# ChaissonLab/LRA

Measured on AMD Instinct MI355X. Metric: aligned Gbp/s, 30 kb ONT vs GRCh38 (MapRead_lowacc end to end incl. SAM text), per job, higher is better.
Workload: dtype int32

## Files before the change

### lra_amd/csrc/sdp.h

```cpp
#pragma once
#include "common.h"
#include <vector>

namespace lra_sdp {

constexpr int LV = 18;
constexpr uint32_t NONE = 0xFFFFFFFFu;
constexpr int MAXALN = 16;
constexpr int PEN_TAB_WG = 4096, PEN_TAB_WAVE = 2048;
constexpr int TRACE_CAP = 2560;

struct PwlTab { long long stops[25]; float slope[25], inter[25]; int c1, c2; };

struct Ent { long long val; int b; float v; };
struct Node {
  uint32_t dBase;
  uint32_t nD, nE;
  int32_t last;
  uint32_t sTop, nBlk;
  uint32_t stkOff, blkOff;
  uint32_t stkCap, blkCap;
  long long eLast;
};

struct ReadArena { uint64_t base; uint32_t entOff, apOff, stkOff, visOff, blkPair, poolPair, poolPairs, edOff, visPl; };

struct PtArgs {
  uint64_t nc;
  const uint64_t* cluster_off; const uint64_t* c_start; const uint32_t* c_count; const int32_t* c_strand;
  const uint32_t* q; const uint32_t* t; const int32_t* len;
  const uint32_t* clusRead; const uint64_t* clusFragOff; const uint64_t* clusPtOff; const uint64_t* fragOff; const uint64_t* ptOff;
  const float* rate_in; float rate; int single;
  uint32_t* fq; uint32_t* ft; int32_t* flen; uint32_t* fcl; uint32_t* fai; float* fval; uint32_t* fprevNode; uint32_t* fprevInd; uint8_t* fflags;
  uint8_t* used; uint8_t* fstrand;
  const uint32_t* qe; const uint32_t* te; uint32_t* fqe; uint32_t* fte;
  uint64_t* key1; uint32_t* pay1; uint32_t* iq; uint32_t* it; uint8_t* ifl; uint32_t* ifr; uint32_t* ptRead;
};

struct BuildArgs {
  int r0, n;
  const uint32_t* order;
  const uint64_t* ptOff;
  const uint32_t* hq; const uint32_t* ht; const uint8_t* hfl; const uint32_t* h2; const uint64_t* key3; const uint32_t* pay3;
  uint32_t* scratch;
  uint32_t* cntEntries; uint32_t* cntNodes; uint32_t* cntD; uint32_t* cntV; uint32_t* cntRC;
  uint32_t* lines;
  const ReadArena* ra;
  uint32_t* status;
  unsigned long long* stat;
};

struct ProcArgs {
  int r0, n;
  const uint32_t* order;
  const uint64_t* ptOff; const uint64_t* fragOff;
  const uint8_t* hfl; const uint32_t* hfr;
  const int32_t* flen; float* fval; uint32_t* fprevNode; uint32_t* fprevInd; uint8_t* fflags;
  const float* rate_in; float rate;
  const ReadArena* ra; uint32_t* poolUsed;
  uint32_t* status;
  PwlTab pwl;
  const short* penTab; int penN;
  int dbg;
  int wgNoRing;
  char* wgScratch; const uint64_t* wgOff;
  unsigned long long* stat;
};

struct TraceArgs {
  int r0, n, numAln, single; float alnthres;
  int boxes, globalK; const uint32_t* fqe; const uint32_t* fte; const int32_t* numAnchors; int32_t* chainNum;
  const uint64_t* fragOff; const uint64_t* read_off;
  const uint32_t* fq; const uint32_t* ft; const int32_t* flen; const uint32_t* fcl; const uint32_t* fai;
  const float* fval; const uint32_t* fpred; const uint8_t* fflags; const uint32_t* opay;
  uint8_t* used;
  const ReadArena* ra;
  uint32_t* nChains; uint64_t* chainStart; uint32_t* chainLen; uint32_t* chainBox; float* chainValue;
  uint32_t* ccl; uint32_t* can; uint8_t* clink; uint32_t* cq; uint32_t* ct; int32_t* clen; uint8_t* cstrand; const uint8_t* fstrand;
  const uint32_t* status;
};

namespace {
__device__ __forceinline__ void wave_sync() {
  __builtin_amdgcn_fence(__ATOMIC_RELEASE, "workgroup");
// ... 124 lines not shown
```

### lra_amd/csrc/sdp.hip

```cpp
#include "sdp.h"
#include "scan.h"
#include <algorithm>
#include <cmath>
#include <cstring>
#include <cstdlib>
#include <vector>

using namespace lra_sdp;

namespace {

inline size_t sz(size_t n, size_t elem) { return (n * elem + 255) / 256 * 256; }
inline char* take(char*& w, size_t n, size_t e) { char* p = w; w += sz(n, e); return p; }
#define SDP_TRY(call) do { const int rc__ = (call); if (rc__) return rc__; } while (0)

static long sdp_big_points(const lra_ctx* ctx, int mode) {
  if (const char* e = getenv("LRA_SDP_BIG_POINTS")) return atol(e);
  if (ctx->sdp_inner) return 1500;
  if (mode == 0) return 2500;
  return ctx->pipelined ? 14000 : 6000;
}

int pwl_table(Call& c) {
  lra_ctx* ctx = c.ctx; hipStream_t st = c.st; const lra_sdp_opts* opts = c.opts; PwlTab& pw = c.pw;
// ... 41 lines not shown
  c.fragOff = (uint64_t*)take(wa, n1, 8); c.ptOff = (uint64_t*)take(wa, n1, 8);
  c.status = (uint32_t*)take(wa, n1, 4); c.nChains = (uint32_t*)take(wa, n1, 4);
  c.chainStart = (uint64_t*)take(wa, nslot, 8); c.chainLen = (uint32_t*)take(wa, nslot, 4); c.chainValue = (float*)take(wa, nslot, 4);
  c.chainBox = (uint32_t*)take(wa, 4 * nslot, 4);
  c.chainNum = (int32_t*)take(wa, nslot, 4);
  LRA_HIP_CHECK(ctx, hipMemsetAsync(c.chainLen, 0, nslot * 4, st));
  if (NC > 0) {
    lra_time_begin(ctx, ctx->sdp_inner ? "sdp_inner_points" : "sdp_points");
    launch_cluster_counts(st, NC, c.boxes ? nullptr : c.d_c_count, c.clusFragCnt, c.clusPtCnt, opts->mode == LRA_SDP_SINGLE_CLUSTER);
    lra_time_end(ctx);
  }
  SDP_TRY(lra_exclusive_scan<uint32_t>(ctx, (long)NC, c.clusFragCnt, c.clusFragOff));
  SDP_TRY(lra_exclusive_scan<uint32_t>(ctx, (long)NC, c.clusPtCnt, c.clusPtOff));
  launch_read_offsets(st, n_reads, c.d_cluster_off, c.clusFragOff, c.clusPtOff, c.fragOff, c.ptOff, c.clusRead, c.status, c.nChains);
  c.h_frag.resize(n1); c.h_pt.resize(n1);
  LRA_HIP_CHECK(ctx, hipMemcpyAsync(c.h_frag.data(), c.fragOff, n1 * 8, hipMemcpyDeviceToHost, st));
  LRA_HIP_CHECK(ctx, hipMemcpyAsync(c.h_pt.data(), c.ptOff, n1 * 8, hipMemcpyDeviceToHost, st));
  LRA_HIP_CHECK(ctx, hipStreamSynchronize(st));
  const uint64_t NF = c.NF = c.h_frag[n_reads], NP = c.NP = c.h_pt[n_reads];
  out->n_frags = NF; out->n_points = NP;
  size_t needF = sz(NF + 1, 4) * 16 + sz(2 * NF + 2, 4) + sz(NF + 1, 1) * 5 + sz(NF + 1, 8) * 2 + 4096;
  char* wf = (char*)lra_ensure(ctx, 8, needF);
  if (!wf) return LRA_ERR_NOMEM;
  c.fq = (uint32_t*)take(wf, NF + 1, 4); c.ft = (uint32_t*)take(wf, NF + 1, 4); c.flen = (int32_t*)take(wf, NF + 1, 4);
  c.fcl = (uint32_t*)take(wf, NF + 1, 4); c.fai = (uint32_t*)take(wf, NF + 1, 4); c.fval = (float*)take(wf, NF + 1, 4);
  c.fprevNode = (uint32_t*)take(wf, NF + 1, 4); c.fprevInd = (uint32_t*)take(wf, NF + 1, 4);
  c.ccl = (uint32_t*)take(wf, NF + 1, 4); c.can = (uint32_t*)take(wf, NF + 1, 4);
  c.fflags = (uint8_t*)take(wf, NF + 1, 1); c.used = (uint8_t*)take(wf, NF + 1, 1); c.clink = (uint8_t*)take(wf, NF + 1, 1);
  c.fstrand = (uint8_t*)take(wf, NF + 1, 1); c.cstrand = (uint8_t*)take(wf, NF + 1, 1);
  c.cq = (uint32_t*)take(wf, NF + 1, 4); c.ct = (uint32_t*)take(wf, NF + 1, 4); c.clen = (int32_t*)take(wf, NF + 1, 4);
  c.okey = (uint64_t*)take(wf, NF + 1, 8);
  c.fqe = (uint32_t*)take(wf, NF + 1, 4); c.fte = (uint32_t*)take(wf, NF + 1, 4);
  size_t needP = sz(NP + 1, 8) * 3 + sz(NP + 1, 4) * 11 + sz(NP + 1, 1) * 2 + sz(NF + 1, 4) * 2 + 4096;
  char* wp = (char*)lra_ensure(ctx, 9, needP);
  if (!wp) return LRA_ERR_NOMEM;
  c.key1 = (uint64_t*)take(wp, NP + 1, 8); c.key2 = (uint64_t*)take(wp, NP + 1, 8); c.key3 = (uint64_t*)take(wp, NP + 1, 8);
  c.pay1 = (uint32_t*)take(wp, NP + 1, 4); c.pay2 = (uint32_t*)take(wp, NP + 1, 4); c.pay3 = (uint32_t*)take(wp, NP + 1, 4);
  c.iq = (uint32_t*)take(wp, NP + 1, 4); c.it = (uint32_t*)take(wp, NP + 1, 4); c.ifr = (uint32_t*)take(wp, NP + 1, 4);
  c.ptRead = (uint32_t*)take(wp, NP + 1, 4);
  c.hq = (uint32_t*)take(wp, NP + 1, 4); c.ht = (uint32_t*)take(wp, NP + 1, 4); c.hfr = (uint32_t*)take(wp, NP + 1, 4);
  c.spare = (uint32_t*)take(wp, NP + 1, 4);
  c.ifl = (uint8_t*)take(wp, NP + 1, 1); c.hfl = (uint8_t*)take(wp, NP + 1, 1);
  c.opay = (uint32_t*)take(wp, NF + 1, 4); c.fragRead = (uint32_t*)take(wp, NF + 1, 4);
  out->d_n_chains = c.nChains; out->d_chain_start = c.chainStart; out->d_chain_len = c.chainLen; out->d_chain_box = c.chainBox; out->d_chain_value = c.chainValue;
  out->d_chain_cluster = c.ccl; out->d_chain_anchor = c.can; out->d_chain_link = c.clink; out->d_chain_q = c.cq; out->d_chain_t = c.ct; out->d_chain_alen = c.clen;
  out->d_chain_strand = c.cstrand; out->d_frag_off = c.fragOff; out->d_frag_val = c.fval; out->d_status = c.status;
  out->d_chain_num_anchors = c.boxes ? c.chainNum : nullptr;
  return LRA_OK;
}

void make_points(const Call& c) {
  lra_ctx* ctx = c.ctx; const lra_sdp_opts* opts = c.opts;
  PtArgs pa;
  pa.nc = c.NC; pa.cluster_off = c.d_cluster_off; pa.c_start = c.d_c_start; pa.c_count = c.d_c_count; pa.c_strand = c.d_c_strand; pa.q = c.d_q; pa.t = c.d_t; pa.len = c.d_len;
  pa.clusRead = c.clusRead; pa.clusFragOff = c.clusFragOff; pa.clusPtOff = c.clusPtOff; pa.fragOff = c.fragOff; pa.ptOff = c.ptOff; pa.rate_in = c.d_rate; pa.rate = opts->rate; pa.single = opts->mode == LRA_SDP_SINGLE_CLUSTER;
  pa.fq = c.fq; pa.ft = c.ft; pa.flen = c.flen; pa.fcl = c.fcl; pa.fai = c.fai; pa.fval = c.fval; pa.fprevNode = c.fprevNode; pa.fprevInd = c.fprevInd; pa.fflags = c.fflags; pa.used = c.used; pa.fstrand = c.fstrand;
  pa.qe = c.d_qe; pa.te = c.d_te; pa.fqe = c.fqe; pa.fte = c.fte;
  pa.key1 = c.key1; pa.pay1 = c.pay1; pa.iq = c.iq; pa.it = c.it; pa.ifl = c.ifl; pa.ifr = c.ifr; pa.ptRead = c.ptRead;
  lra_time_begin(ctx, ctx->sdp_inner ? "sdp_inner_points" : "sdp_points");
  launch_points(c.st, pa);
  launch_frag_read(c.st, c.n_reads, c.fragOff, c.fragRead);
  lra_time_end(ctx);
}

int sort_points(const Call& c) {
  lra_ctx* ctx = c.ctx; hipStream_t st = c.st; const int n_reads = c.n_reads; const uint64_t NP = c.NP;
  SDP_TRY(lra_sort_mostly_unique_batch(ctx, n_reads, c.ptOff, NP, c.key1, c.pay1, c.key3, c.pay3, 64, c.sort));
  lra_time_begin(ctx, ctx->sdp_inner ? "sdp_inner_points" : "sdp_points");
  launch_gather(st, NP, c.ptRead, c.ptOff, c.pay1, c.iq, c.it, c.ifl, c.ifr, c.hq, c.ht, c.hfl, c.hfr, c.key2, c.pay2, c.key3, c.pay3);
  lra_time_end(ctx);
  SDP_TRY(lra_sort_mostly_unique_batch(ctx, n_reads, c.ptOff, NP, c.key2, c.pay2, c.key1, c.pay1, 63, c.sort));
  lra_time_begin(ctx, c.sort.tag);
  const int rc = lra_segsort_pairs_scratch(ctx, c.key3, c.key1, c.pay3, c.pay1, NP, (uint64_t)n_reads, c.ptOff, c.ptOff + 1, 0, 42);
  lra_time_end(ctx);
  if (rc) return rc;
  LRA_HIP_CHECK(ctx, hipGetLastError());
  return LRA_OK;
}

int chunk_begin(const Call& c, Chunk& k) {
  lra_ctx* ctx = c.ctx; hipStream_t st = c.st; const std::vector<uint64_t>& h_pt = c.h_pt;
  const int r0 = k.r0, nr = k.nr; const uint64_t cp = k.cp;
  const size_t nr1 = (size_t)nr + 1;
  size_t needS = sz(34 * cp + 64 * (size_t)nr + 64, 4) + sz(nr1, 4) * 8 + sz(2 * nr1, 4) + sz(nr1 + 1, 8) * 3 + sz(nr1, sizeof(ReadArena)) + 4096;
  char* ws = (char*)lra_ensure(ctx, 10, needS);
  if (!ws) return LRA_ERR_NOMEM;
  k.scratch = (uint32_t*)take(ws, 34 * cp + 64 * (size_t)nr + 64, 4);
  k.cntE = (uint32_t*)take(ws, nr1, 4); k.cntN = (uint32_t*)take(ws, nr1, 4); k.cntD = (uint32_t*)take(ws, nr1, 4);
  k.cntV = (uint32_t*)take(ws, nr1, 4); k.cntRC = (uint32_t*)take(ws, nr1, 4); k.order = (uint32_t*)take(ws, nr1, 4); k.order2 = (uint32_t*)take(ws, nr1, 4); k.poolUsed = (uint32_t*)take(ws, nr1, 4);
  k.lines = (uint32_t*)take(ws, 2 * nr1, 4);
  LRA_HIP_CHECK(ctx, hipMemsetAsync(k.lines, 0, 2 * nr1 * 4, st));
  {
    std::vector<uint32_t> h_order(nr);
    uint64_t maxP = 0;
    for (int i = 0; i < nr; i++) maxP = std::max<uint64_t>(maxP, h_pt[r0 + i + 1] - h_pt[r0 + i]);
    if (maxP <= (uint64_t(1) << 24)) {
      std::vector<uint32_t> at(maxP + 2, 0);
      for (int i = 0; i < nr; i++) at[maxP - (h_pt[r0 + i + 1] - h_pt[r0 + i]) + 1]++;
      for (uint64_t v = 1; v <= maxP + 1; v++) at[v] += at[v - 1];
      for (int i = 0; i < nr; i++) h_order[at[maxP - (h_pt[r0 + i + 1] - h_pt[r0 + i])]++] = (uint32_t)i;
    } else {
      for (int i = 0; i < nr; i++) h_order[i] = (uint32_t)i;
      std::sort(h_order.begin(), h_order.end(), [&](uint32_t x, uint32_t y) {
        const uint64_t px = h_pt[r0 + x + 1] - h_pt[r0 + x], py = h_pt[r0 + y + 1] - h_pt[r0 + y];
        return px != py ? px > py : x < y;
      });
    }
    LRA_HIP_CHECK(ctx, hipMemcpyAsync(k.order, h_order.data(), (size_t)nr * 4, hipMemcpyHostToDevice, st));
    LRA_HIP_CHECK(ctx, hipStreamSynchronize(st));
    k.h_orderAll = h_order;
  }
  take(ws, nr1 + 1, 8);
  k.bytes = (uint64_t*)take(ws, nr1 + 1, 8); k.byteOff = (uint64_t*)take(ws, nr1 + 1, 8);
  k.ra = (ReadArena*)take(ws, nr1, sizeof(ReadArena));
  BuildArgs& ba = k.ba;
  memset(&ba, 0, sizeof ba);
  ba.r0 = r0; ba.n = nr; ba.ptOff = c.ptOff; ba.hq = c.hq; ba.ht = c.ht; ba.hfl = c.hfl; ba.h2 = c.pay2; ba.key3 = c.key1; ba.pay3 = c.pay1; ba.scratch = k.scratch;
  ba.cntEntries = k.cntE; ba.cntNodes = k.cntN; ba.cntD = k.cntD; ba.cntV = k.cntV; ba.cntRC = k.cntRC; ba.lines = k.lines; ba.status = c.status; ba.order = k.order; ba.stat = nullptr;
  if (diag_build_stat()) { k.buildStat.alloc(16, st); ba.stat = k.buildStat.d; }
  k.h_status.assign(nr, 0);
  k.subOrder = k.order; k.nsub = nr;
  return LRA_OK;
}

void count_pass(const Call& c, const Chunk& k, const uint32_t* d_ord, const std::vector<uint32_t>& h_ord, int n) {
  lra_ctx* ctx = c.ctx; hipStream_t st = c.st; const lra_sdp_opts* opts = c.opts; const std::vector<uint64_t>& h_pt = c.h_pt; const int r0 = k.r0;
  lra_time_begin(ctx, ctx->sdp_inner ? "sdp_inner_build_count" : "sdp_build_count");
  const long big_pts = sdp_big_points(ctx, opts->mode);
  int nb0 = 0;
  while (nb0 < n && (long)(h_pt[r0 + h_ord[nb0] + 1] - h_pt[r0 + h_ord[nb0]]) >= big_pts) nb0++;
  const bool forked = nb0 > 0 && n > nb0;
  BuildArgs bc = k.ba; bc.order = d_ord; bc.n = n;
  if (nb0 > 0) launch_wg_builds(false, forked ? lra_side_fork(ctx) : st, bc, nb0);
  if (n > nb0) launch_small_builds(false, ctx, bc, d_ord, h_ord, h_pt.data() + r0, nb0, n);
  if (forked) lra_side_join(ctx);
  lra_time_end(ctx);
}

int read_rc(const Call& c, Chunk& k) {
  lra_ctx* ctx = c.ctx; hipStream_t st = c.st; const int nr = k.nr;
  std::vector<uint32_t> h_rc(nr), h_e(nr);
  LRA_HIP_CHECK(ctx, hipMemcpyAsync(h_rc.data(), k.cntRC, (size_t)nr * 4, hipMemcpyDeviceToHost, st));
  LRA_HIP_CHECK(ctx, hipMemcpyAsync(h_e.data(), k.onePass ? k.cntV : k.cntE, (size_t)nr * 4, hipMemcpyDeviceToHost, st));
  LRA_HIP_CHECK(ctx, hipStreamSynchronize(st));
  k.maxRC = 0; k.totE = 0;
  for (uint32_t v : h_rc) k.maxRC = std::max(k.maxRC, v);
  for (uint32_t v : h_e) k.totE += v;
  return LRA_OK;
}

int chunk_sizes(const Call& c, Chunk& k) {
  const lra_sdp_opts* opts = c.opts; const int nr = k.nr;
  const bool onePassEnv = !(getenv("LRA_SDP_ONEPASS") && getenv("LRA_SDP_ONEPASS")[0] == '0');
  k.onePass = onePassEnv && !getenv("LRA_SDP_RATIOS");
  if (!k.onePass) { count_pass(c, k, k.order, k.h_orderAll, nr); SDP_TRY(read_rc(c, k)); }
  else {
    float fE = opts->mode == 0 ? 10.0f : 8.5f, fN = 2.0f;
    if (const char* e = getenv("LRA_SDP_ESTIMATE")) { float x = 0, y = 0; if (sscanf(e, "%f,%f", &x, &y) == 2 && x > 0 && y > 0) { fE = x; fN = y; } }
    launch_arena_estimate(c.st, nr, k.r0, c.ptOff, fE, fN, k.cntE, k.cntN, k.cntD);
  }
  diag_ratios(c, k);
  return LRA_OK;
}

void pick_large_reads(const Call& c, const Chunk& k, Attempt& a) {
  lra_ctx* ctx = c.ctx; const lra_sdp_opts* opts = c.opts; const std::vector<uint64_t>& h_pt = c.h_pt; const std::vector<uint32_t>& ordAtt = *a.ordAtt;
  const int r0 = k.r0, nsub = k.nsub, att = a.att; const bool onePass = k.onePass, dbg = a.dbg;
  int nbig = 0;
  {
    const long big_pts = sdp_big_points(ctx, opts->mode);
// ... 229 lines not shown
```

### lra_amd/csrc/sdp_build.hip

```cpp
#include "sdp.h"
#include <type_traits>

using namespace lra_sdp;

namespace {

template <int NW>
__device__ __forceinline__ int blk_incl_scan(int v, int lane, int wave, int* s_w, int& total) {
  const int inc = wave_incl_scan(v, lane);
  if (NW == 1) { total = __builtin_amdgcn_readlane(inc, 63); return inc; }
  if (lane == 63) s_w[wave] = inc;
  __syncthreads();
  int pre = 0, tot = 0;
#pragma unroll
  for (int w = 0; w < NW; w++) { const int x = s_w[w]; tot += x; if (w < wave) pre += x; }
  __syncthreads();
  total = tot;
  return inc + pre;
}
template <bool EMIT, int NW, int MODE = 0, int OCC = 8, bool BSTAT = false>
__global__ void __launch_bounds__(64 * NW, NW == 1 ? OCC : 1) sdp_build(BuildArgs a) {
  constexpr int NT = 64 * NW;
  constexpr bool LDSV = MODE == 1, NARROW = MODE != 0;
  using IT = typename std::conditional<NARROW, uint16_t, uint32_t>::type;
  using DT = typename std::conditional<NARROW, uint32_t, long long>::type;
  constexpr IT INONE = (IT)~(IT)0;
  extern __shared__ __attribute__((aligned(16))) char dyn_lds[];
  __shared__ int s_w[4][NW == 1 ? 1 : NW];
  __shared__ unsigned long long s_bt[BSTAT ? 8 : 1];
  unsigned long long btPrev = 0;
  constexpr bool bstat = BSTAT;
  if (bstat) { if (threadIdx.x < 8) s_bt[threadIdx.x] = 0; btPrev = __builtin_amdgcn_s_memtime(); }
#define BTICK(k_) do { if (bstat) { const unsigned long long t__ = __builtin_amdgcn_s_memtime(); if (threadIdx.x == 0) s_bt[k_] += t__ - btPrev; btPrev = t__; } } while (0)
  const int rr = (int)a.order[blockIdx.x], r = a.r0 + rr, tid = threadIdx.x, lane = tid & 63, wave = tid >> 6;
  auto SYNC = [&]() { if (NW == 1) wave_sync(); else __syncthreads(); };
  const uint64_t p0 = a.ptOff[r], pc0 = a.ptOff[a.r0];
  const int P = (int)(a.ptOff[r + 1] - p0);
  if (P == 0) { if (tid == 0) { if (!EMIT) { a.cntEntries[rr] = 0; a.cntNodes[rr] = 0; a.cntD[rr] = 0; } a.cntV[rr] = 0; a.cntRC[rr] = 0; } return; }
  const uint32_t* hq = a.hq + p0; const uint32_t* ht = a.ht + p0; const uint32_t* h2 = a.h2 + p0;
  const uint64_t* key3 = a.key3 + p0; const uint32_t* pay3 = a.pay3 + p0;
  uint32_t* S = a.scratch + 34 * (p0 - pc0) + 64 * (uint64_t)rr;
  const int NCAP = P + 2;
  uint32_t* tbl = S + 8 * P + 2;
  uint32_t* tmp = tbl + 12 * NCAP;
  IT* eb_ = LDSV ? (IT*)dyn_lds : (IT*)S;
  IT* rowOf = eb_; IT* colOf = rowOf + P;
  IT* lp = colOf + P;
  IT* ln = lp + 2 * P;
  IT* pf = ln + 2 * P;
  IT* ph = pf + P + 1;
  IT* ll = NARROW ? ph + P + 1 : (IT*)(tmp + 8 * NCAP);
  DT* ld = LDSV ? (DT*)(dyn_lds + ((((size_t)(10 * P + 2) * sizeof(IT)) + 7) & ~(size_t)7)) : NARROW ? (DT*)(tmp + 8 * NCAP) : (DT*)(ll + 2 * P);
  auto LN = [&](int idx) -> uint32_t { const IT v = ln[idx]; return v == INONE ? NONE : (uint32_t)v; };
#define TB(c, f, k) tbl[((c) * 6 + (f)) * NCAP + (k)]
#define TM(f, k) tmp[(f) * NCAP + (k)]
  enum { F_LS, F_LE, F_SB, F_SE, F_EB, F_EE };
  enum { T_C1S, T_C1E, T_ND, T_NE, T_CH0, T_CH1, T_BASE, T_GID };
  int R = 0, C = 0;
  for (int i0 = 0; i0 < P; i0 += NT) {
    const int i = i0 + tid;
    const int head = (i < P) && (i == 0 || hq[i] != hq[i - 1]);
    int tot; const int inc = blk_incl_scan<NW>(head, lane, wave, s_w[0], tot);
    if (i < P) rowOf[i] = R + inc - 1;
    R += tot;
  }
  for (int i0 = 0; i0 < P; i0 += NT) {
    const int i = i0 + tid;
    const int head = (i < P) && (i == 0 || ht[h2[i]] != ht[h2[i - 1]]);
    int tot; const int inc = blk_incl_scan<NW>(head, lane, wave, s_w[0], tot);
    if (i < P) colOf[h2[i]] = C + inc - 1;
    C += tot;
  }
  int cOff[5];
  {
    int c0 = 0, c1 = 0, c2 = 0, c3 = 0;
    for (int i = tid; i < P; i += NT) { const int cl = (int)(key3[i] >> 40); c0 += cl == 0; c1 += cl == 1; c2 += cl == 2; c3 += cl == 3; }
    for (int o = 32; o > 0; o >>= 1) { c0 += __shfl_xor(c0, o); c1 += __shfl_xor(c1, o); c2 += __shfl_xor(c2, o); c3 += __shfl_xor(c3, o); }
    if (NW > 1) {
      if (lane == 0) { s_w[0][wave] = c0; s_w[1][wave] = c1; s_w[2][wave] = c2; s_w[3][wave] = c3; }
      __syncthreads();
      c0 = c1 = c2 = c3 = 0;
      for (int w = 0; w < NW; w++) { c0 += s_w[0][w]; c1 += s_w[1][w]; c2 += s_w[2][w]; c3 += s_w[3][w]; }
      __syncthreads();
    }
    c0 = __builtin_amdgcn_readfirstlane(c0); c1 = __builtin_amdgcn_readfirstlane(c1); c2 = __builtin_amdgcn_readfirstlane(c2);
    cOff[0] = 0; cOff[1] = c0; cOff[2] = c0 + c1; cOff[3] = c0 + c1 + c2; cOff[4] = P;
  }
  SYNC();
  BTICK(0);
  uint32_t nEntries = 0, nNodesTot = 0, sumD = 0, nVisits = 0;
  Node* nodesR = nullptr; Ent* entR = nullptr; uint32_t* apR = nullptr; int2* stkR = nullptr; uint2* visR = nullptr; long long* edR = nullptr;
  uint32_t blkPair = 0, visPl = 0;
  if (EMIT) {
    const ReadArena A = a.ra[rr];
    char* b = arena_ptr(A.base);
    blkPair = A.blkPair; visPl = A.visPl;
    nodesR = (Node*)b; entR = (Ent*)(b + A.entOff); apR = (uint32_t*)(b + A.apOff); stkR = (int2*)(b + A.stkOff); visR = (uint2*)(b + A.visOff);
    edR = (long long*)(b + A.edOff);
  }
  bool overflow = false, outgrown = false;
  const uint64_t capE = EMIT ? a.cntEntries[rr] : 0, capN = EMIT ? a.cntNodes[rr] : 0, capD = EMIT ? a.cntD[rr] : 0;
  for (int fam = 0; fam < 4 && !outgrown; fam++) {
    const bool col = fam & 1, back = fam >= 2, desc = (fam == 1 || fam == 2), swapped = (fam == 3);
    const IT* lineOf = col ? colOf : rowOf;
    const int nLines = col ? C : R;
    const int sc = back ? 2 : 0;
    const int nS = cOff[sc + 1] - cOff[sc], nEn = cOff[sc + 2] - cOff[sc + 1], Pf = nS + nEn;
    if (nS == 0 || nEn == 0) continue;
    const int fam2 = fam & 1;
    const int nPl = EMIT ? (int)(fam2 ? visPl >> 8 : visPl & 0xffu) : LV;
    uint2* visF = EMIT ? visR + (size_t)(fam2 ? visPl & 0xffu : 0u) * P : nullptr;
    const int dSide = swapped ? 1 : 0, eSide = swapped ? 0 : 1;
    for (int i = tid; i < Pf; i += NT) {
      const uint32_t pos = pay3[cOff[sc] + i];
      lp[i] = (IT)pos; ln[i] = 0; ll[i] = lineOf[pos];
      ld[i] = (DT)(back ? (long long)ht[pos] + hq[pos] : (long long)ht[pos] - hq[pos]);
    }
    if (tid == 0) { TB(0, F_LS, 0) = 0; TB(0, F_LE, 0) = nLines; TB(0, F_SB, 0) = 0; TB(0, F_SE, 0) = nS; TB(0, F_EB, 0) = nS; TB(0, F_EE, 0) = Pf; }
    int nNodes = 1, cur = 0;
    SYNC();
    BTICK(7);
    for (int level = 0; nNodes > 0 && !outgrown; level++) {
      if (level >= nPl) { overflow = true; break; }
      uint2* visL = EMIT ? visF + (size_t)level * P : nullptr;
      const int nxt = cur ^ 1;
      IT* lpc = lp + cur * P; IT* lpn = lp + nxt * P;
      IT* llc = ll + cur * P; IT* lln = ll + nxt * P;
      DT* ldc = ld + (size_t)cur * P; DT* ldn = ld + (size_t)nxt * P;
      {
        int carry = 0;
        constexpr int UA = 4;
        for (int i0 = 0; i0 < Pf; i0 += UA * NT) {
          uint32_t kk[UA]; uint32_t ss[UA], ee[UA]; IT lv[UA]; int ff[UA];
#pragma unroll
          for (int u = 0; u < UA; u++) { const int i = i0 + u * NT + tid; kk[u] = i < Pf ? LN(i) : NONE; lv[u] = i < Pf ? llc[i] : (IT)0; }
#pragma unroll
          for (int u = 0; u < UA; u++) { ss[u] = 0; ee[u] = 0; if (kk[u] != NONE) { ss[u] = TB(cur, F_LS, kk[u]); ee[u] = TB(cur, F_LE, kk[u]); } }
#pragma unroll
          for (int u = 0; u < UA; u++) ff[u] = kk[u] == NONE ? 0 : (ee[u] - ss[u] > 1) ? (lv[u] < ((ss[u] + ee[u]) >> 1)) : 1;
#pragma unroll
          for (int u = 0; u < UA; u++) {
            const int i = i0 + u * NT + tid;
            if (i0 + u * NT >= Pf) break;
            int tot; const int inc = blk_incl_scan<NW>(ff[u], lane, wave, s_w[0], tot);
            if (i < Pf) pf[i] = (IT)(carry + inc - ff[u]);
            carry += tot;
          }
        }
        if (tid == 0) pf[Pf] = (IT)carry;
      }
      SYNC();
      BTICK(1);
      for (int k = tid; k < nNodes; k += NT) {
        TM(T_C1S, k) = (uint32_t)pf[TB(cur, F_SE, k)] - (uint32_t)pf[TB(cur, F_SB, k)];
        TM(T_C1E, k) = (uint32_t)pf[TB(cur, F_EE, k)] - (uint32_t)pf[TB(cur, F_EB, k)];
      }
      SYNC();
      {
        constexpr int UC = 2;
        for (int i0 = 0; i0 < Pf; i0 += UC * NT) {
          uint32_t kk[UC], pi0[UC], pi1[UC], sb[UC], c1[UC], psb[UC]; IT vlp[UC], vll[UC]; DT vld[UC];
#pragma unroll
          for (int u = 0; u < UC; u++) {
            const int i = i0 + u * NT + tid;
            kk[u] = NONE; pi0[u] = 0; pi1[u] = 0; vlp[u] = 0; vll[u] = 0; vld[u] = 0;
            if (i < Pf) { kk[u] = LN(i); pi0[u] = (uint32_t)pf[i]; pi1[u] = (uint32_t)pf[i + 1]; vlp[u] = lpc[i]; vll[u] = llc[i]; vld[u] = ldc[i]; }
          }
#pragma unroll
          for (int u = 0; u < UC; u++) {
            const int i = i0 + u * NT + tid;
            const bool isS = i < nS;
            sb[u] = 0; c1[u] = 0;
            if (kk[u] != NONE) { sb[u] = isS ? TB(cur, F_SB, kk[u]) : TB(cur, F_EB, kk[u]); c1[u] = isS ? TM(T_C1S, kk[u]) : TM(T_C1E, kk[u]); }
          }
#pragma unroll
          for (int u = 0; u < UC; u++) psb[u] = kk[u] != NONE ? (uint32_t)pf[sb[u]] : 0;
#pragma unroll
          for (int u = 0; u < UC; u++) {
            const int i = i0 + u * NT + tid;
            if (i >= Pf) continue;
            if (kk[u] == NONE) { ln[P + i] = INONE; continue; }
            const uint32_t rank1 = pi0[u] - psb[u];
            const uint32_t first = pi1[u] - pi0[u];
            const uint32_t np_ = first ? sb[u] + rank1 : sb[u] + c1[u] + ((uint32_t)i - sb[u] - rank1);
            lpn[np_] = vlp[u]; lln[np_] = vll[u]; ldn[np_] = vld[u];
            ln[P + np_] = (IT)(2 * kk[u] + (first ? 0 : 1));
          }
        }
      }
      SYNC();
      BTICK(2);
      {
        int carry = 0;
        constexpr int UD = NW == 1 ? 4 : 2;
        for (int j0 = 0; j0 < Pf; j0 += UD * NT) {
          uint32_t k2v[UD], le[UD], ls[UD], bg[UD], c1[UD]; DT d0[UD], d1[UD]; int hd[UD];
#pragma unroll
          for (int u = 0; u < UD; u++) {
            const int j = j0 + u * NT + tid;
            k2v[u] = NONE; d0[u] = 0; d1[u] = 0;
            if (j < Pf) { k2v[u] = LN(P + j); d0[u] = ldn[j]; d1[u] = j > 0 ? ldn[j - 1] : ldn[j]; }
          }
#pragma unroll
          for (int u = 0; u < UD; u++) {
            const int j = j0 + u * NT + tid;
            const bool isS = j < nS;
            le[u] = 0; ls[u] = 0; bg[u] = 0; c1[u] = 0;
            if (k2v[u] != NONE) {
              const uint32_t k = k2v[u] >> 1;
              le[u] = TB(cur, F_LE, k); ls[u] = TB(cur, F_LS, k); bg[u] = isS ? TB(cur, F_SB, k) : TB(cur, F_EB, k); c1[u] = isS ? TM(T_C1S, k) : TM(T_C1E, k);
            }
          }
#pragma unroll
          for (int u = 0; u < UD; u++) {
            const int j = j0 + u * NT + tid;
            hd[u] = 0;
            if (k2v[u] != NONE) {
              const uint32_t side = k2v[u] & 1;
              const bool isS = j < nS;
              const bool leaf = le[u] - ls[u] == 1;
              const bool in = leaf || (int)side == (isS ? eSide : dSide);
              if (in) {
                uint32_t beg = bg[u];
                if (!leaf && side == 1) beg += c1[u];
                hd[u] = ((uint32_t)j == beg) ? 1 : (d0[u] != d1[u]);
              }
            }
          }
#pragma unroll
          for (int u = 0; u < UD; u++) {
            const int j = j0 + u * NT + tid;
            if (j0 + u * NT >= Pf) break;
            int tot; const int inc = blk_incl_scan<NW>(hd[u], lane, wave, s_w[0], tot);
            if (j < Pf) ph[j] = (IT)(carry + inc - hd[u]);
            carry += tot;
          }
        }
        if (tid == 0) ph[Pf] = (IT)carry;
      }
      SYNC();
      BTICK(3);
      int nNext = 0;
      for (int k0 = 0; k0 < nNodes; k0 += NT) {
        const int k = k0 + tid;
        uint32_t nD = 0, nE = 0, act0 = 0, act1 = 0, full = 0;
        uint32_t ls = 0, le = 0, sb = 0, se = 0, eb = 0, ee = 0, c1S = 0, c1E = 0;
        bool leaf = false;
        if (k < nNodes) {
          ls = TB(cur, F_LS, k); le = TB(cur, F_LE, k); sb = TB(cur, F_SB, k); se = TB(cur, F_SE, k); eb = TB(cur, F_EB, k); ee = TB(cur, F_EE, k);
          c1S = TM(T_C1S, k); c1E = TM(T_C1E, k);
          leaf = le - ls == 1;
          uint32_t dB, dE, eB, eE;
          if (leaf) { dB = eb; dE = ee; eB = sb; eE = se; }
          else {
            dB = dSide == 0 ? eb : eb + c1E; dE = dSide == 0 ? eb + c1E : ee;
            eB = eSide == 0 ? sb : sb + c1S; eE = eSide == 0 ? sb + c1S : se;
          }
          nD = (uint32_t)ph[dE] - (uint32_t)ph[dB]; nE = (uint32_t)ph[eE] - (uint32_t)ph[eB];
          full = nD > 0 && nE > 0;
          if (!leaf) {
            const bool goD = nD > 0, goE = nE > 0;
            if (dSide == 0) { act0 = goD; act1 = goE; } else { act1 = goD; act0 = goE; }
          }
        }
        int totF, totEnt, totD, totC;
        const int incF = blk_incl_scan<NW>((int)full, lane, wave, s_w[0], totF), incEnt = blk_incl_scan<NW>((int)(full ? nD + nE : 0), lane, wave, s_w[1], totEnt),
                  incD = blk_incl_scan<NW>((int)(full ? nD : 0), lane, wave, s_w[2], totD), incC = blk_incl_scan<NW>((int)(act0 + act1), lane, wave, s_w[3], totC);
        if (EMIT && ((uint64_t)nNodesTot + totF > capN || (uint64_t)nEntries + totEnt > capE || (uint64_t)sumD + totD > capD)) { outgrown = true; break; }
        if (k < nNodes) {
          const uint32_t gid = nNodesTot + incF - full, base = nEntries + incEnt - (full ? nD + nE : 0), dpre = sumD + incD - (full ? nD : 0);
          TM(T_ND, k) = nD; TM(T_NE, k) = nE; TM(T_GID, k) = full ? gid : NONE; TM(T_BASE, k) = base;
          uint32_t ci = nNext + incC - (act0 + act1);
          const uint32_t med = (ls + le) >> 1;
          TM(T_CH0, k) = NONE; TM(T_CH1, k) = NONE;
          if (act0) { TM(T_CH0, k) = ci; TB(nxt, F_LS, ci) = ls; TB(nxt, F_LE, ci) = med; TB(nxt, F_SB, ci) = sb; TB(nxt, F_SE, ci) = sb + c1S;
                      TB(nxt, F_EB, ci) = eb; TB(nxt, F_EE, ci) = eb + c1E; ci++; }
          if (act1) { TM(T_CH1, k) = ci; TB(nxt, F_LS, ci) = med; TB(nxt, F_LE, ci) = le; TB(nxt, F_SB, ci) = sb + c1S; TB(nxt, F_SE, ci) = se;
                      TB(nxt, F_EB, ci) = eb + c1E; TB(nxt, F_EE, ci) = ee; }
          if (EMIT && full) {
            Node nd;
            nd.dBase = base; nd.nD = nD; nd.nE = nE; nd.last = -1; nd.sTop = 1; nd.nBlk = 0;
            nd.stkOff = 2 * dpre + 4 * gid; nd.blkOff = blkPair + 2 * base + 8 * gid; nd.stkCap = 2 * nD + 4; nd.blkCap = 2 * (nD + nE) + 8;
            nd.eLast = 0;
            nodesR[gid] = nd;
            stkR[nd.stkOff] = make_int2(-1, (int)nE + 1);
          }
        }
        nNodesTot += totF; nEntries += totEnt; sumD += totD; nNext += totC;
      }
      if (outgrown) break;
      SYNC();
      BTICK(4);
      {
        constexpr int UF = 2;
        for (int j0 = 0; j0 < Pf; j0 += UF * NT) {
          uint32_t k2v[UF], le[UF], ls[UF], ch[UF], gidv[UF], bg[UF], c1[UF], nNE[UF], nND[UF], bs[UF], p0v[UF], p1v[UF], pbg[UF], posv[UF], tq[UF], tt[UF];
#pragma unroll
          for (int u = 0; u < UF; u++) {
            const int j = j0 + u * NT + tid;
            k2v[u] = NONE; p0v[u] = 0; p1v[u] = 0; posv[u] = 0;
            if (j < Pf) { k2v[u] = LN(P + j); if (EMIT) { p0v[u] = (uint32_t)ph[j]; p1v[u] = (uint32_t)ph[j + 1]; posv[u] = lpn[j]; } }
          }
#pragma unroll
          for (int u = 0; u < UF; u++) {
            const int j = j0 + u * NT + tid;
            const bool isS = j < nS;
            le[u] = 0; ls[u] = 0; ch[u] = 0; gidv[u] = NONE; bg[u] = 0; c1[u] = 0; nNE[u] = 0; nND[u] = 0; bs[u] = 0; tq[u] = 0; tt[u] = 0;
            if (k2v[u] != NONE) {
              const uint32_t k = k2v[u] >> 1, side = k2v[u] & 1;
              le[u] = TB(cur, F_LE, k); ls[u] = TB(cur, F_LS, k); ch[u] = side == 0 ? TM(T_CH0, k) : TM(T_CH1, k); gidv[u] = TM(T_GID, k);
              if (EMIT) {
                bg[u] = isS ? TB(cur, F_SB, k) : TB(cur, F_EB, k); c1[u] = isS ? TM(T_C1S, k) : TM(T_C1E, k);
                nNE[u] = TM(T_NE, k); nND[u] = TM(T_ND, k); bs[u] = TM(T_BASE, k);
                tq[u] = hq[posv[u]]; tt[u] = ht[posv[u]];
              }
            }
          }
#pragma unroll
          for (int u = 0; u < UF; u++) {
            pbg[u] = 0;
            if (EMIT && k2v[u] != NONE) {
              const uint32_t side = k2v[u] & 1;
              const bool leaf = le[u] - ls[u] == 1;
              uint32_t beg = bg[u];
              if (!leaf && side == 1) beg += c1[u];
              bg[u] = beg;
              pbg[u] = (uint32_t)ph[beg];
            }
          }
#pragma unroll
          for (int u = 0; u < UF; u++) {
            const int j = j0 + u * NT + tid;
            if (j >= Pf) continue;
            if (k2v[u] == NONE) { ln[j] = INONE; continue; }
            const uint32_t side = k2v[u] & 1;
            const bool leaf = le[u] - ls[u] == 1;
            ln[j] = (IT)(leaf ? NONE : ch[u]);
            const uint32_t gid = gidv[u];
            const bool isS = j < nS;
            const bool in = leaf || (int)side == (isS ? eSide : dSide);
            if (in && gid != NONE) {
              if (!EMIT) nVisits++;
              else {
                const uint32_t head = p1v[u] - p0v[u];
                const uint32_t grp = p0v[u] - pbg[u] + head - 1;
                const uint32_t n = isS ? nNE[u] : nND[u];
                const uint32_t idx = desc ? n - 1 - grp : grp;
                const uint32_t ent = bs[u] + (isS ? nND[u] + idx : idx);
                const uint32_t pos = posv[u];
                if (head) {
                  const long long dgv = back ? (long long)tt[u] + tq[u] : (long long)tt[u] - tq[u];
                  entR[ent].val = dgv;
                  if (isS && idx == n - 1) nodesR[gid].eLast = dgv;
                }
                visL[pos] = make_uint2(gid, idx);
              }
            }
          }
        }
      }
      SYNC();
      BTICK(5);
      if (EMIT) {
        constexpr int UG = 2;
        for (int j0 = 0; j0 < Pf; j0 += UG * NT) {
          uint32_t k2v[UG], gidv[UG], le[UG], ls[UG], bg[UG], c1[UG], nDv[UG], nEv[UG], bs[UG], p0v[UG], p1v[UG], pbg[UG];
          bool on[UG];
#pragma unroll
          for (int u = 0; u < UG; u++) {
            const int j = j0 + u * NT + tid;
            k2v[u] = NONE; p0v[u] = 0; p1v[u] = 0;
            if (j < Pf) { k2v[u] = LN(P + j); p0v[u] = (uint32_t)ph[j]; p1v[u] = (uint32_t)ph[j + 1]; }
          }
#pragma unroll
          for (int u = 0; u < UG; u++) {
            const int j = j0 + u * NT + tid;
            const bool isS = j < nS;
            gidv[u] = NONE; le[u] = 0; ls[u] = 0; bg[u] = 0; c1[u] = 0; nDv[u] = 0; nEv[u] = 0; bs[u] = 0;
            if (k2v[u] != NONE && p1v[u] != p0v[u]) {
              const uint32_t k = k2v[u] >> 1;
              gidv[u] = TM(T_GID, k); le[u] = TB(cur, F_LE, k); ls[u] = TB(cur, F_LS, k);
              bg[u] = isS ? TB(cur, F_SB, k) : TB(cur, F_EB, k); c1[u] = isS ? TM(T_C1S, k) : TM(T_C1E, k);
              nDv[u] = TM(T_ND, k); nEv[u] = TM(T_NE, k); bs[u] = TM(T_BASE, k);
            }
          }
#pragma unroll
          for (int u = 0; u < UG; u++) {
            const int j = j0 + u * NT + tid;
            const bool isS = j < nS;
            const uint32_t side = k2v[u] & 1;
            const bool leaf = le[u] - ls[u] == 1;
            on[u] = k2v[u] != NONE && p1v[u] != p0v[u] && gidv[u] != NONE && (leaf || (int)side == (isS ? eSide : dSide));
            pbg[u] = 0;
            if (on[u]) { uint32_t beg = bg[u]; if (!leaf && side == 1) beg += c1[u]; pbg[u] = (uint32_t)ph[beg]; }
          }
          uint32_t entv[UG], mv[UG], lo[UG], cnt[UG]; long long xv[UG]; const Ent* opp[UG];
#pragma unroll
          for (int u = 0; u < UG; u++) {
            const int j = j0 + u * NT + tid;
            const bool isS = j < nS;
            const uint32_t grp = p0v[u] - pbg[u];
            const uint32_t n = isS ? nEv[u] : nDv[u];
            const uint32_t idx = desc ? n - 1 - grp : grp;
            entv[u] = bs[u] + (isS ? nDv[u] + idx : idx);
            opp[u] = entR + bs[u] + (isS ? 0 : nDv[u]);
            mv[u] = isS ? nDv[u] : nEv[u];
            xv[u] = on[u] ? entR[entv[u]].val : 0;
            lo[u] = 0; cnt[u] = on[u] ? mv[u] : 0;
          }
          while (true) {
            bool any = false;
#pragma unroll
            for (int u = 0; u < UG; u++) any |= cnt[u] > 0;
            if (!any) break;
            long long vM[UG], vL[UG], vR[UG];
#pragma unroll
            for (int u = 0; u < UG; u++) {
              const uint32_t step = cnt[u] >> 1, it = lo[u] + step, cntT = cnt[u] > 0 ? cnt[u] - step - 1 : 0;
              vM[u] = cnt[u] > 0 ? opp[u][it].val : 0;
              vL[u] = step > 0 ? opp[u][lo[u] + (step >> 1)].val : 0;
              vR[u] = cntT > 0 ? opp[u][it + 1 + (cntT >> 1)].val : 0;
            }
#pragma unroll
            for (int u = 0; u < UG; u++) {
              if (cnt[u] == 0) continue;
              const bool isS = j0 + u * NT + tid < nS;
              auto go = [&](long long v) { return isS ? (desc ? v > xv[u] : v <= xv[u]) : (desc ? v >= xv[u] : v < xv[u]); };
              const uint32_t step = cnt[u] >> 1, it = lo[u] + step;
              if (go(vM[u])) {
                lo[u] = it + 1; cnt[u] -= step + 1;
                if (cnt[u] > 0) { const uint32_t s2 = cnt[u] >> 1; if (go(vR[u])) { lo[u] += s2 + 1; cnt[u] -= s2 + 1; } else cnt[u] = s2; }
              } else {
                cnt[u] = step;
                if (cnt[u] > 0) { const uint32_t s2 = cnt[u] >> 1; if (go(vL[u])) { lo[u] += s2 + 1; cnt[u] -= s2 + 1; } else cnt[u] = s2; }
              }
            }
          }
#pragma unroll
          for (int u = 0; u < UG; u++) {
            if (!on[u]) continue;
            const bool isS = j0 + u * NT + tid < nS;
            const uint32_t ent = entv[u], m = mv[u];
            entR[ent].b = isS ? (int32_t)lo[u] - 1 : (lo[u] == m ? -1 : (int32_t)lo[u]);
            if (!isS) edR[ent] = lo[u] == m ? 0 : opp[u][lo[u]].val;
            entR[ent].v = 0.f; apR[ent] = 0;
          }
        }
      }
      nNodes = nNext; cur = nxt;
      SYNC();
      BTICK(6);
    }
  }
  if (bstat && tid == 0) { for (int k = 0; k < 8; k++) atomicAdd(a.stat + k, s_bt[k]); atomicAdd(a.stat + 8, (unsigned long long)P); }
  for (int o = 32; o > 0; o >>= 1) nVisits += __shfl_xor(nVisits, o);
  if (NW > 1) {
    if (lane == 0) s_w[0][wave] = (int)nVisits;
    __syncthreads();
    nVisits = 0;
    for (int w = 0; w < NW; w++) nVisits += (uint32_t)s_w[0][w];
  }
  if (tid == 0) {
    if (!EMIT) { a.cntEntries[rr] = nEntries; a.cntNodes[rr] = nNodesTot; a.cntD[rr] = sumD; a.cntV[rr] = nVisits; a.cntRC[rr] = (uint32_t)max(R, C); a.lines[2 * rr] = (uint32_t)R; a.lines[2 * rr + 1] = (uint32_t)C; }
    else { a.cntV[rr] = nEntries; a.cntRC[rr] = (uint32_t)max(R, C); }
    if (overflow) atomicOr(&a.status[r], (uint32_t)LRA_ST_RANGE);
    if (outgrown) atomicOr(&a.status[r], (uint32_t)LRA_ST_CAPACITY);
  }
#undef TB
#undef TM
#undef BTICK
}

template <bool EMIT>
void small_builds(lra_ctx* ctx, const BuildArgs& ba, const uint32_t* d_order, const std::vector<uint32_t>& h_order, const uint64_t* h_pt, int from, int to) {
  hipStream_t st = ctx->stream;
  auto pts = [&](int i) { return (long)(h_pt[h_order[i] + 1] - h_pt[h_order[i]]); };
  int at = from;
  const long caps[3] = {512, 256, 128};
  int cut[4];
  for (int c = 0; c < 3; c++) { while (at < to && pts(at) > caps[c]) at++; cut[c] = at; }
  cut[3] = to;
  if (cut[0] > from) {
    int mid = from;
    while (mid < cut[0] && pts(mid) >= 16384) mid++;
    if (mid > from) { BuildArgs bb = ba; bb.order = d_order + from; hipLaunchKernelGGL((sdp_build<EMIT, 1, 0>), dim3(mid - from), dim3(64), 0, st, bb); }
    if (cut[0] > mid) {
      BuildArgs bb = ba; bb.order = d_order + mid;
      const bool occ6 = ctx->pipelined;
      if (bb.stat) { if (occ6) hipLaunchKernelGGL((sdp_build<EMIT, 1, 2, 6, true>), dim3(cut[0] - mid), dim3(64), 0, st, bb); else hipLaunchKernelGGL((sdp_build<EMIT, 1, 2, 8, true>), dim3(cut[0] - mid), dim3(64), 0, st, bb); }
      else if (occ6) hipLaunchKernelGGL((sdp_build<EMIT, 1, 2, 6>), dim3(cut[0] - mid), dim3(64), 0, st, bb);
      else hipLaunchKernelGGL((sdp_build<EMIT, 1, 2>), dim3(cut[0] - mid), dim3(64), 0, st, bb);
    }
  }
  for (int c = 0; c < 3; c++) {
    const int n = cut[c + 1] - cut[c];
    if (n <= 0) continue;
    BuildArgs bb = ba; bb.order = d_order + cut[c];
    hipLaunchKernelGGL((sdp_build<EMIT, 1, 1>), dim3(n), dim3(64), (size_t)(28 * caps[c] + 32), st, bb);
  }
}

}

namespace lra_sdp {

void launch_wg_builds(bool emit, hipStream_t st, const BuildArgs& ba, int n) {
  if (emit) hipLaunchKernelGGL((sdp_build<true, 16>), dim3(n), dim3(1024), 0, st, ba);
  else hipLaunchKernelGGL((sdp_build<false, 16>), dim3(n), dim3(1024), 0, st, ba);
}
void launch_small_builds(bool emit, lra_ctx* ctx, const BuildArgs& ba, const uint32_t* d_order, const std::vector<uint32_t>& h_order, const uint64_t* h_pt, int from, int to) {
  if (emit) small_builds<true>(ctx, ba, d_order, h_order, h_pt, from, to);
  else small_builds<false>(ctx, ba, d_order, h_order, h_pt, from, to);
}

}
```

Before: 1.153.

## Pack SDP build node tables into array-of-structs records

```diff
diff --git a/lra_amd/csrc/sdp.h b/lra_amd/csrc/sdp.h
--- a/lra_amd/csrc/sdp.h
+++ b/lra_amd/csrc/sdp.h
@@ -1,5 +1,6 @@
 #pragma once
 #include "common.h"
+#include "sdp_layout.h"
 #include <vector>
 
 namespace lra_sdp {
diff --git a/lra_amd/csrc/sdp.hip b/lra_amd/csrc/sdp.hip
--- a/lra_amd/csrc/sdp.hip
+++ b/lra_amd/csrc/sdp.hip
@@ -147,10 +147,10 @@
   lra_ctx* ctx = c.ctx; hipStream_t st = c.st; const std::vector<uint64_t>& h_pt = c.h_pt;
   const int r0 = k.r0, nr = k.nr; const uint64_t cp = k.cp;
   const size_t nr1 = (size_t)nr + 1;
-  size_t needS = sz(34 * cp + 64 * (size_t)nr + 64, 4) + sz(nr1, 4) * 8 + sz(2 * nr1, 4) + sz(nr1 + 1, 8) * 3 + sz(nr1, sizeof(ReadArena)) + 4096;
+  size_t needS = sz(build_slot_words(cp, (uint64_t)nr) + 64, 4) + sz(nr1, 4) * 8 + sz(2 * nr1, 4) + sz(nr1 + 1, 8) * 3 + sz(nr1, sizeof(ReadArena)) + 4096;
   char* ws = (char*)lra_ensure(ctx, 10, needS);
   if (!ws) return LRA_ERR_NOMEM;
-  k.scratch = (uint32_t*)take(ws, 34 * cp + 64 * (size_t)nr + 64, 4);
+  k.scratch = (uint32_t*)take(ws, build_slot_words(cp, (uint64_t)nr) + 64, 4);
   k.cntE = (uint32_t*)take(ws, nr1, 4); k.cntN = (uint32_t*)take(ws, nr1, 4); k.cntD = (uint32_t*)take(ws, nr1, 4);
   k.cntV = (uint32_t*)take(ws, nr1, 4); k.cntRC = (uint32_t*)take(ws, nr1, 4); k.order = (uint32_t*)take(ws, nr1, 4); k.order2 = (uint32_t*)take(ws, nr1, 4); k.poolUsed = (uint32_t*)take(ws, nr1, 4);
   k.lines = (uint32_t*)take(ws, 2 * nr1, 4);
diff --git a/lra_amd/csrc/sdp_build.hip b/lra_amd/csrc/sdp_build.hip
--- a/lra_amd/csrc/sdp_build.hip
+++ b/lra_amd/csrc/sdp_build.hip
@@ -4,6 +4,27 @@
 using namespace lra_sdp;
 
 namespace {
+
+template <bool NARROW> struct NodeRec;
+template <> struct NodeRec<true> {
+  using PT = uint32_t;
+  struct alignas(16) Split { PT line, s, e, end; };
+  struct alignas(16) Emit { PT cnt, ch; uint32_t base, gid; };
+  static __device__ __forceinline__ PT pack(uint32_t lo, uint32_t hi) { return (lo & 0xffffu) | hi << 16; }
+  static __device__ __forceinline__ uint32_t lo(PT p) { return p & 0xffffu; }
+  static __device__ __forceinline__ uint32_t hi(PT p) { return p >> 16; }
+  static __device__ __forceinline__ uint32_t child(uint32_t c) { return c == 0xffffu ? NONE : c; }
+};
+template <> struct NodeRec<false> {
+  using PT = uint2;
+  struct alignas(16) Split { PT line, s, e, end; };
+  struct alignas(8) Emit { PT cnt, ch; uint32_t base, gid; };
+  static __device__ __forceinline__ PT pack(uint32_t lo, uint32_t hi) { return make_uint2(lo, hi); }
+  static __device__ __forceinline__ uint32_t lo(PT p) { return p.x; }
+  static __device__ __forceinline__ uint32_t hi(PT p) { return p.y; }
+  static __device__ __forceinline__ uint32_t child(uint32_t c) { return c; }
+};
+static_assert(sizeof(NodeRec<true>::Split) == 16 && sizeof(NodeRec<true>::Emit) == 16 && sizeof(NodeRec<false>::Split) == 32 && sizeof(NodeRec<false>::Emit) == 24, "sdp_layout.h");
 
 template <int NW>
 __device__ __forceinline__ int blk_incl_scan(int v, int lane, int wave, int* s_w, int& total) {
@@ -39,23 +60,21 @@
   if (P == 0) { if (tid == 0) { if (!EMIT) { a.cntEntries[rr] = 0; a.cntNodes[rr] = 0; a.cntD[rr] = 0; } a.cntV[rr] = 0; a.cntRC[rr] = 0; } return; }
   const uint32_t* hq = a.hq + p0; const uint32_t* ht = a.ht + p0; const uint32_t* h2 = a.h2 + p0;
   const uint64_t* key3 = a.key3 + p0; const uint32_t* pay3 = a.pay3 + p0;
-  uint32_t* S = a.scratch + 34 * (p0 - pc0) + 64 * (uint64_t)rr;
+  char* S = (char*)(a.scratch + build_slot_words(p0 - pc0, (uint64_t)rr));
   const int NCAP = P + 2;
-  uint32_t* tbl = S + 8 * P + 2;
-  uint32_t* tmp = tbl + 12 * NCAP;
-  IT* eb_ = LDSV ? (IT*)dyn_lds : (IT*)S;
-  IT* rowOf = eb_; IT* colOf = rowOf + P;
-  IT* lp = colOf + P;
-  IT* ln = lp + 2 * P;
-  IT* pf = ln + 2 * P;
-  IT* ph = pf + P + 1;
-  IT* ll = NARROW ? ph + P + 1 : (IT*)(tmp + 8 * NCAP);
-  DT* ld = LDSV ? (DT*)(dyn_lds + ((((size_t)(10 * P + 2) * sizeof(IT)) + 7) & ~(size_t)7)) : NARROW ? (DT*)(tmp + 8 * NCAP) : (DT*)(ll + 2 * P);
+  const BuildLayout lay = build_layout((uint64_t)P, MODE);
+  using Rec = NodeRec<NARROW>; using PT = typename Rec::PT; using SplitRec = typename Rec::Split; using EmitRec = typename Rec::Emit;
+  SplitRec* split = (SplitRec*)(S + lay.split);
+  EmitRec* emit = (EmitRec*)(S + lay.emit);
+  char* eb_ = LDSV ? dyn_lds : S + lay.elem;
+  IT* rowOf = (IT*)(eb_ + lay.rowOf); IT* colOf = (IT*)(eb_ + lay.colOf);
+  IT* lp = (IT*)(eb_ + lay.lp);
+  IT* ln = (IT*)(eb_ + lay.ln);
+  IT* pf = (IT*)(eb_ + lay.pf);
+  IT* ph = (IT*)(eb_ + lay.ph);
+  IT* ll = (IT*)(eb_ + lay.ll);
+  DT* ld = (DT*)(eb_ + lay.ld);
   auto LN = [&](int idx) -> uint32_t { const IT v = ln[idx]; return v == INONE ? NONE : (uint32_t)v; };
-#define TB(c, f, k) tbl[((c) * 6 + (f)) * NCAP + (k)]
-#define TM(f, k) tmp[(f) * NCAP + (k)]
-  enum { F_LS, F_LE, F_SB, F_SE, F_EB, F_EE };
-  enum { T_C1S, T_C1E, T_ND, T_NE, T_CH0, T_CH1, T_BASE, T_GID };
   int R = 0, C = 0;
   for (int i0 = 0; i0 < P; i0 += NT) {
     const int i = i0 + tid;
@@ -116,7 +135,7 @@
       lp[i] = (IT)pos; ln[i] = 0; ll[i] = lineOf[pos];
       ld[i] = (DT)(back ? (long long)ht[pos] + hq[pos] : (long long)ht[pos] - hq[pos]);
     }
-    if (tid == 0) { TB(0, F_LS, 0) = 0; TB(0, F_LE, 0) = nLines; TB(0, F_SB, 0) = 0; TB(0, F_SE, 0) = nS; TB(0, F_EB, 0) = nS; TB(0, F_EE, 0) = Pf; }
+    if (tid == 0) { SplitRec root; root.line = Rec::pack(0, nLines); root.s = Rec::pack(0, 0); root.e = Rec::pack(nS, 0); root.end = Rec::pack(nS, Pf); split[0] = root; }
     int nNodes = 1, cur = 0;
     SYNC();
     BTICK(7);
@@ -127,6 +146,7 @@
       IT* lpc = lp + cur * P; IT* lpn = lp + nxt * P;
       IT* llc = ll + cur * P; IT* lln = ll + nxt * P;
       DT* ldc = ld + (size_t)cur * P; DT* ldn = ld + (size_t)nxt * P;
+      const SplitRec* spc = split + (size_t)cur * NCAP; SplitRec* spn = split + (size_t)nxt * NCAP;
       {
         int carry = 0;
         constexpr int UA = 4;
@@ -135,7 +155,7 @@
 #pragma unroll
           for (int u = 0; u < UA; u++) { const int i = i0 + u * NT + tid; kk[u] = i < Pf ? LN(i) : NONE; lv[u] = i < Pf ? llc[i] : (IT)0; }
 #pragma unroll
-          for (int u = 0; u < UA; u++) { ss[u] = 0; ee[u] = 0; if (kk[u] != NONE) { ss[u] = TB(cur, F_LS, kk[u]); ee[u] = TB(cur, F_LE, kk[u]); } }
+          for (int u = 0; u < UA; u++) { ss[u] = 0; ee[u] = 0; if (kk[u] != NONE) { const PT l = spc[kk[u]].line; ss[u] = Rec::lo(l); ee[u] = Rec::hi(l); } }
 #pragma unroll
           for (int u = 0; u < UA; u++) ff[u] = kk[u] == NONE ? 0 : (ee[u] - ss[u] > 1) ? (lv[u] < ((ss[u] + ee[u]) >> 1)) : 1;
 #pragma unroll
@@ -152,8 +172,11 @@
       SYNC();
       BTICK(1);
       for (int k = tid; k < nNodes; k += NT) {
-        TM(T_C1S, k) = (uint32_t)pf[TB(cur, F_SE, k)] - (uint32_t)pf[TB(cur, F_SB, k)];
-        TM(T_C1E, k) = (uint32_t)pf[TB(cur, F_EE, k)] - (uint32_t)pf[TB(cur, F_EB, k)];
+        SplitRec* rec = split + (size_t)cur * NCAP + k;
+        const PT s = rec->s, e = rec->e, end = rec->end;
+        const uint32_t sb = Rec::lo(s), eb = Rec::lo(e);
+        rec->s = Rec::pack(sb, (uint32_t)pf[Rec::lo(end)] - (uint32_t)pf[sb]);
+        rec->e = Rec::pack(eb, (uint32_t)pf[Rec::hi(end)] - (uint32_t)pf[eb]);
       }
       SYNC();
       {
@@ -171,7 +194,7 @@
             const int i = i0 + u * NT + tid;
             const bool isS = i < nS;
             sb[u] = 0; c1[u] = 0;
-            if (kk[u] != NONE) { sb[u] = isS ? TB(cur, F_SB, kk[u]) : TB(cur, F_EB, kk[u]); c1[u] = isS ? TM(T_C1S, kk[u]) : TM(T_C1E, kk[u]); }
+            if (kk[u] != NONE) { const PT h = *(isS ? &spc[kk[u]].s : &spc[kk[u]].e); sb[u] = Rec::lo(h); c1[u] = Rec::hi(h); }
           }
 #pragma unroll
           for (int u = 0; u < UC; u++) psb[u] = kk[u] != NONE ? (uint32_t)pf[sb[u]] : 0;
@@ -208,7 +231,8 @@
             le[u] = 0; ls[u] = 0; bg[u] = 0; c1[u] = 0;
             if (k2v[u] != NONE) {
               const uint32_t k = k2v[u] >> 1;
-              le[u] = TB(cur, F_LE, k); ls[u] = TB(cur, F_LS, k); bg[u] = isS ? TB(cur, F_SB, k) : TB(cur, F_EB, k); c1[u] = isS ? TM(T_C1S, k) : TM(T_C1E, k);
+              const PT l = spc[k].line, h = *(isS ? &spc[k].s : &spc[k].e);
+              le[u] = Rec::hi(l); ls[u] = Rec::lo(l); bg[u] = Rec::lo(h); c1[u] = Rec::hi(h);
             }
           }
 #pragma unroll
@@ -247,8 +271,8 @@
         uint32_t ls = 0, le = 0, sb = 0, se = 0, eb = 0, ee = 0, c1S = 0, c1E = 0;
         bool leaf = false;
         if (k < nNodes) {
-          ls = TB(cur, F_LS, k); le = TB(cur, F_LE, k); sb = TB(cur, F_SB, k); se = TB(cur, F_SE, k); eb = TB(cur, F_EB, k); ee = TB(cur, F_EE, k);
-          c1S = TM(T_C1S, k); c1E = TM(T_C1E, k);
+          const SplitRec rec = spc[k];
+          ls = Rec::lo(rec.line); le = Rec::hi(rec.line); sb = Rec::lo(rec.s); c1S = Rec::hi(rec.s); eb = Rec::lo(rec.e); c1E = Rec::hi(rec.e); se = Rec::lo(rec.end); ee = Rec::hi(rec.end);
           leaf = le - ls == 1;
           uint32_t dB, dE, eB, eE;
           if (leaf) { dB = eb; dE = ee; eB = sb; eE = se; }
@@ -269,14 +293,12 @@
         if (EMIT && ((uint64_t)nNodesTot + totF > capN || (uint64_t)nEntries + totEnt > capE || (uint64_t)sumD + totD > capD)) { outgrown = true; break; }
         if (k < nNodes) {
           const uint32_t gid = nNodesTot + incF - full, base = nEntries + incEnt - (full ? nD + nE : 0), dpre = sumD + incD - (full ? nD : 0);
-          TM(T_ND, k) = nD; TM(T_NE, k) = nE; TM(T_GID, k) = full ? gid : NONE; TM(T_BASE, k) = base;
           uint32_t ci = nNext + incC - (act0 + act1);
           const uint32_t med = (ls + le) >> 1;
-          TM(T_CH0, k) = NONE; TM(T_CH1, k) = NONE;
-          if (act0) { TM(T_CH0, k) = ci; TB(nxt, F_LS, ci) = ls; TB(nxt, F_LE, ci) = med; TB(nxt, F_SB, ci) = sb; TB(nxt, F_SE, ci) = sb + c1S;
-                      TB(nxt, F_EB, ci) = eb; TB(nxt, F_EE, ci) = eb + c1E; ci++; }
-          if (act1) { TM(T_CH1, k) = ci; TB(nxt, F_LS, ci) = med; TB(nxt, F_LE, ci) = le; TB(nxt, F_SB, ci) = sb + c1S; TB(nxt, F_SE, ci) = se;
-                      TB(nxt, F_EB, ci) = eb + c1E; TB(nxt, F_EE, ci) = ee; }
+          uint32_t ch0 = NONE, ch1 = NONE;
+          if (act0) { ch0 = ci; SplitRec c; c.line = Rec::pack(ls, med); c.s = Rec::pack(sb, 0); c.e = Rec::pack(eb, 0); c.end = Rec::pack(sb + c1S, eb + c1E); spn[ci] = c; ci++; }
+          if (act1) { ch1 = ci; SplitRec c; c.line = Rec::pack(med, le); c.s = Rec::pack(sb + c1S, 0); c.e = Rec::pack(eb + c1E, 0); c.end = Rec::pack(se, ee); spn[ci] = c; }
+          { EmitRec m; m.cnt = Rec::pack(nD, nE); m.ch = Rec::pack(ch0, ch1); m.base = base; m.gid = full ? gid : NONE; emit[k] = m; }
           if (EMIT && full) {
             Node nd;
             nd.dBase = base; nd.nD = nD; nd.nE = nE; nd.last = -1; nd.sTop = 1; nd.nBlk = 0;
@@ -308,10 +330,12 @@
             le[u] = 0; ls[u] = 0; ch[u] = 0; gidv[u] = NONE; bg[u] = 0; c1[u] = 0; nNE[u] = 0; nND[u] = 0; bs[u] = 0; tq[u] = 0; tt[u] = 0;
             if (k2v[u] != NONE) {
               const uint32_t k = k2v[u] >> 1, side = k2v[u] & 1;
-              le[u] = TB(cur, F_LE, k); ls[u] = TB(cur, F_LS, k); ch[u] = side == 0 ? TM(T_CH0, k) : TM(T_CH1, k); gidv[u] = TM(T_GID, k);
+              const PT l = spc[k].line; const EmitRec m = emit[k];
+              le[u] = Rec::hi(l); ls[u] = Rec::lo(l); ch[u] = Rec::child(side == 0 ? Rec::lo(m.ch) : Rec::hi(m.ch)); gidv[u] = m.gid;
               if (EMIT) {
-                bg[u] = isS ? TB(cur, F_SB, k) : TB(cur, F_EB, k); c1[u] = isS ? TM(T_C1S, k) : TM(T_C1E, k);
-                nNE[u] = TM(T_NE, k); nND[u] = TM(T_ND, k); bs[u] = TM(T_BASE, k);
+                const PT h = *(isS ? &spc[k].s : &spc[k].e);
+                bg[u] = Rec::lo(h); c1[u] = Rec::hi(h);
+                nNE[u] = Rec::hi(m.cnt); nND[u] = Rec::lo(m.cnt); bs[u] = m.base;
                 tq[u] = hq[posv[u]]; tt[u] = ht[posv[u]];
               }
             }
@@ -379,9 +403,10 @@
             gidv[u] = NONE; le[u] = 0; ls[u] = 0; bg[u] = 0; c1[u] = 0; nDv[u] = 0; nEv[u] = 0; bs[u] = 0;
             if (k2v[u] != NONE && p1v[u] != p0v[u]) {
               const uint32_t k = k2v[u] >> 1;
-              gidv[u] = TM(T_GID, k); le[u] = TB(cur, F_LE, k); ls[u] = TB(cur, F_LS, k);
-              bg[u] = isS ? TB(cur, F_SB, k) : TB(cur, F_EB, k); c1[u] = isS ? TM(T_C1S, k) : TM(T_C1E, k);
-              nDv[u] = TM(T_ND, k); nEv[u] = TM(T_NE, k); bs[u] = TM(T_BASE, k);
+              const PT l = spc[k].line, h = *(isS ? &spc[k].s : &spc[k].e); const EmitRec m = emit[k];
+              gidv[u] = m.gid; le[u] = Rec::hi(l); ls[u] = Rec::lo(l);
+              bg[u] = Rec::lo(h); c1[u] = Rec::hi(h);
+              nDv[u] = Rec::lo(m.cnt); nEv[u] = Rec::hi(m.cnt); bs[u] = m.base;
             }
           }
 #pragma unroll
@@ -466,8 +491,6 @@
     if (overflow) atomicOr(&a.status[r], (uint32_t)LRA_ST_RANGE);
     if (outgrown) atomicOr(&a.status[r], (uint32_t)LRA_ST_CAPACITY);
   }
-#undef TB
-#undef TM
 #undef BTICK
 }
 
diff --git a/lra_amd/csrc/sdp_layout.h b/lra_amd/csrc/sdp_layout.h
--- /dev/null
+++ b/lra_amd/csrc/sdp_layout.h
@@ -0,0 +1,46 @@
+#pragma once
+#include <stdint.h>
+
+#if defined(__HIPCC__) || defined(__CUDACC__)
+#define LRA_SDP_HD __host__ __device__
+#else
+#define LRA_SDP_HD
+#endif
+
+namespace lra_sdp {
+
+constexpr uint64_t BUILD_WORDS_PER_POINT = 36, BUILD_WORDS_PER_READ = 64;
+
+struct BuildLayout {
+  uint64_t split, emit;
+  uint64_t elem;
+  uint64_t rowOf, colOf, lp, ln, pf, ph, ll, ld;
+  uint64_t elemBytes;
+  uint64_t slotBytes;
+};
+
+LRA_SDP_HD inline BuildLayout build_layout(uint64_t P, int mode) {
+  const bool narrow = mode != 0, lds = mode == 1;
+  const uint64_t ncap = P + 2, it = narrow ? 2 : 4, dt = narrow ? 4 : 8, splitB = narrow ? 16 : 32, emitB = narrow ? 16 : 24;
+  BuildLayout L;
+  L.split = 0;
+  L.emit = 2 * ncap * splitB;
+  const uint64_t recEnd = L.emit + ncap * emitB;
+  L.elem = lds ? 0 : recEnd;
+  uint64_t o = 0;
+  L.rowOf = o; o += P * it;
+  L.colOf = o; o += P * it;
+  L.lp = o; o += 2 * P * it;
+  L.ln = o; o += 2 * P * it;
+  L.pf = o; o += (P + 1) * it;
+  L.ph = o; o += (P + 1) * it;
+  L.ll = o; o += 2 * P * it;
+  o = (o + 7) & ~(uint64_t)7;
+  L.ld = o; o += 2 * P * dt;
+  L.elemBytes = o;
+  L.slotBytes = lds ? recEnd : recEnd + o;
+  return L;
+}
+LRA_SDP_HD inline uint64_t build_slot_words(uint64_t points, uint64_t reads) { return BUILD_WORDS_PER_POINT * points + BUILD_WORDS_PER_READ * reads; }
+
+}
```

New measurement: 1.142. 0.99x the previous value.
